# vigor-nf/vigor

Measured on AMD Instinct MI355X. Metric: Mpackets/s device-resident, 64B vignat @1M flows; %HBM roofline, higher is better.
Workload: dtype u8; 1 GPU; vignat 64B, 1M flows, 1xMI355X (parse+hash+map-probe kernel, checksum rewrite); flows=1048576, batch_packets_per_gpu=16777216, global_batch_packets=16777216, frame_bytes=60, slot_bytes=64, order=rr, port=one per burst (vp_dev_batch.in_port), parallelism=single

## Files before the change

vigor_amd/csrc/vp_internal.h:

```cpp
#pragma once

#include <hip/hip_ext.h>
#include <hip/hip_runtime.h>
#include <stdint.h>
#include <stdlib.h>
#include <string.h>

#include <mutex>
#include <tuple>
#include <vector>

#include "../../include/vigpath.h"
#include "vp_device.h"

#define VP_HIP(call)                                                      \
  do {                                                                    \
    hipError_t e_ = (call);                                               \
    if (e_ != hipSuccess) return vp::hip_fail(e_, #call, __FILE__, __LINE__); \
  } while (0)

#define VP_TRY(call)          \
  do {                        \
    int rc_ = (call);         \
    if (rc_) return rc_;      \
// ... 111 lines not shown
  uint32_t sh_live;
  uint32_t own_new;
  uint32_t run_tiles;
  uint32_t last_first;
};

constexpr int kPubGath = 5;
struct CtlPub {
  Ctl ctl;
  uint32_t xtra[(kPubGath + 1) * 64];
  uint32_t epoch;
};

struct JournalCtl {
  uint32_t tail, cnt;
  int64_t floor;
};
constexpr int64_t kJournalNone = INT64_MAX;

struct FlowTable {
  Bucket *bk = nullptr;
  uint32_t bmask = 0;
  uint32_t cap = 0;
  uint32_t mix = 0;
  uint64_t ins_since = 0;
  uint32_t layout_tries = 0;
  uint64_t rebuilds = 0;
  uint32_t *lin = nullptr;
  uint32_t lin_ok = 0;
  bool lin_tried = false;
  uint64_t nb_nominal = 0;
  uint64_t nb_base = 0;
  uint32_t *slot_of = nullptr;
  uint32_t *hash_of = nullptr;
  uint64_t *ts = nullptr;
  uint64_t *tseq = nullptr;
  uint64_t *birth = nullptr;
  uint32_t *stack = nullptr;
  uint32_t *lastg = nullptr;
  Ctl *ctl = nullptr;
  Ctl h_ctl{};
  Ctl *h_pin = nullptr;
  CtlPub *h_pub = nullptr;
  CtlPub *d_pub = nullptr;
  uint32_t pub_epoch = 0;
  uint32_t *ttotal = nullptr;
  uint64_t ts_floor = UINT64_MAX;
  uint32_t fs_hint = 0;
  bool runs_seen = true;
  uint32_t last_run_tiles = 0;
  bool ctl_clean = false;
  uint64_t *ekey = nullptr, *ekey2 = nullptr;
  uint32_t *eidx = nullptr, *eidx2 = nullptr;
  JournalCtl *jr = nullptr;
  uint4 *jrec = nullptr;
  uint32_t jr_n = 0;
  bool jr_on = false;
  uint4 *kv = nullptr;
  uint32_t own_n = 0, own_r = 0;
};

struct CallBuf {
  void *p = nullptr;
  size_t bytes = 0;
  hipEvent_t ev = nullptr;
  hipStream_t last = nullptr;
  bool used = false;
};
int callbuf_reserve(CallBuf &w, size_t bytes, hipStream_t s);
inline int callbuf_done(CallBuf &w, hipStream_t s) {
  VP_HIP(hipEventRecord(w.ev, s));
  w.used = true;
  w.last = s;
  return 0;
}

struct Workspace {
  uint32_t cap_n = 0;
  uint32_t *miss = nullptr;
  uint32_t *miss_sorted = nullptr;
  uint32_t *defer = nullptr;
  uint32_t *reprobe = nullptr;
  uint32_t *reprobe_cnt = nullptr;
  uint32_t *missq = nullptr;
  uint32_t *mkey = nullptr;
  uint32_t *pairs = nullptr;
  uint16_t *in_fill = nullptr;
  size_t in_fill_n = 0;
  CallBuf tx_cnt, txp_sum, rxu_sum, rxm_rec;
  unsigned long long *nkset = nullptr;
  size_t nkset_n = 0;
  uint32_t nk_tag = 0;
  uint32_t *nkbits = nullptr, *nkpre = nullptr, *nkfirst = nullptr, *nkcnt = nullptr;
  size_t nkbits_n = 0, nkfirst_n = 0;
  uint4 *mkq = nullptr;
  uint32_t *mhq = nullptr;
  uint32_t *mhash = nullptr;
  uint32_t *first = nullptr;
  uint32_t *rank = nullptr;
  uint32_t *rep = nullptr;
  uint32_t *assign = nullptr;
  uint32_t *scratch = nullptr;
  uint32_t *log = nullptr;
  uint32_t *log2 = nullptr;
  uint32_t *defer_sorted = nullptr;
  uint32_t *aux = nullptr, *aux_sorted = nullptr;
// ... 252 lines not shown
```

vigor_amd/csrc/vp_table.hip:

```cpp
#include <hip/hip_runtime.h>

#include <cstddef>
#include <hipcub/hipcub.hpp>
#include <unistd.h>

#include <algorithm>
#include <cstdio>
#include <cstdlib>
#include <cstring>
#include <mutex>
#include <vector>

#include "vp_comm.h"
#include "vp_table.h"

namespace vp {

VP_PRELOAD_UNIT(table)


uint32_t grid_for(uint64_t n, uint32_t block, uint32_t max_blocks) {
  uint64_t g = (n + block - 1) / block;
  if (g == 0) g = 1;
  return (uint32_t)(g < max_blocks ? g : max_blocks);
// ... 62 lines not shown
  return 0;
}

int read_ctl_wait(vp_ctx *c, FlowTable &t) {
  hipError_t e;
  while ((e = hipEventQuery(c->evc)) == hipErrorNotReady) {
  }
  VP_HIP(e);
  t.h_ctl = *t.h_pin;
  return 0;
}

int read_ctl2_post(vp_ctx *c, FlowTable &a, FlowTable &b) {
  VP_HIP(hipMemcpyAsync(a.h_pin, a.ctl, sizeof(Ctl), hipMemcpyDeviceToHost,
                        c->stream));
  VP_HIP(hipMemcpyAsync(b.h_pin, b.ctl, sizeof(Ctl), hipMemcpyDeviceToHost,
                        c->stream));
  VP_HIP(hipEventRecord(c->evc, c->stream));
  return 0;
}

int read_ctl2_wait(vp_ctx *c, FlowTable &a, FlowTable &b) {
  hipError_t e;
  while ((e = hipEventQuery(c->evc)) == hipErrorNotReady) {
  }
  VP_HIP(e);
  a.h_ctl = *a.h_pin;
  b.h_ctl = *b.h_pin;
  return 0;
}

int read_ctl2(vp_ctx *c, FlowTable &a, FlowTable &b) {
  VP_HIP(hipMemcpyAsync(a.h_pin, a.ctl, sizeof(Ctl), hipMemcpyDeviceToHost,
                        c->stream));
  VP_HIP(hipMemcpyAsync(b.h_pin, b.ctl, sizeof(Ctl), hipMemcpyDeviceToHost,
                        c->stream));
  VP_HIP(stream_wait(c->stream));
  a.h_ctl = *a.h_pin;
  b.h_ctl = *b.h_pin;
  return 0;
}

TableDev tbl_dev(const FlowTable &t) {
  return TableDev{t.bk,  t.bmask, t.cap,   t.mix, t.slot_of, t.hash_of, t.ts,
                  t.tseq, t.birth, t.stack, t.ctl, t.kv,      t.own_n,   t.own_r,
                  t.lin};
}

template <class T>
static int dalloc(T **p, size_t count) {
  if (count == 0) count = 1;
  hipError_t e = hipMalloc((void **)p, sizeof(T) * count);
  return e == hipSuccess ? 0 : hip_fail(e, "hipMalloc", __FILE__, __LINE__);
}

static int tbl_rebuild(vp_ctx *c, FlowTable &t, uint64_t nb_new = 0);
static int tbl_choose_layout(vp_ctx *c, FlowTable &t);
static int tbl_try_linear(vp_ctx *c, FlowTable &t);
__global__ void lay_count(TableDev t, uint32_t mix, uint32_t *cnt);
__global__ void lay_score(const uint32_t *cnt, uint32_t nb, uint32_t *over);

static uint64_t tbl_entries(const FlowTable &t) {
  return (uint64_t)(t.bmask + 1) * kBucketEntries;
}

uint32_t tbl_initial_mix() {
  const char *mix = getenv("VIGPATH_MIX");
  return mix && atoi(mix) ? kMixMul : 0;
}

int tbl_alloc(vp_ctx *c, FlowTable &t, uint32_t cap) {
  (void)c;
  uint64_t nb = 64;
  while (nb < cap) nb <<= 1;
  t.nb_base = nb;
  int k = 1;
  if (const char *sp = getenv("VIGPATH_SPARSE")) k = atoi(sp);
  if (k > 0) nb <<= std::min(k, 3);
  if (k < 0) nb = std::max<uint64_t>(64, nb >> std::min(-k, 3));
  t.bmask = (uint32_t)(nb - 1);
  t.nb_nominal = nb;
  t.cap = cap;
  t.mix = tbl_initial_mix();
  VP_TRY(dalloc(&t.bk, nb));
  VP_TRY(dalloc(&t.slot_of, cap));
  VP_TRY(dalloc(&t.hash_of, cap));
  VP_TRY(dalloc(&t.ts, cap));
  VP_TRY(dalloc(&t.tseq, cap));
  VP_TRY(dalloc(&t.birth, cap));
  VP_TRY(dalloc(&t.stack, cap));
  VP_TRY(dalloc(&t.lastg, cap));
  VP_TRY(dalloc(&t.ctl, 1));
  VP_HIP(hipHostMalloc((void **)&t.h_pin, sizeof(Ctl), hipHostMallocDefault));
  VP_HIP(hipHostMalloc((void **)&t.h_pub, sizeof(CtlPub),
                       hipHostMallocMapped | hipHostMallocCoherent));
  memset(t.h_pub, 0, sizeof(CtlPub));
  VP_HIP(hipHostGetDevicePointer((void **)&t.d_pub, t.h_pub, 0));
  VP_TRY(dalloc(&t.ttotal, 1));
  VP_TRY(dalloc(&t.ekey, cap));
  VP_TRY(dalloc(&t.ekey2, cap));
  VP_TRY(dalloc(&t.eidx, cap));
  VP_TRY(dalloc(&t.eidx2, cap));
  VP_HIP(hipMemset(t.bk, 0xFF, sizeof(Bucket) * nb));
  VP_HIP(hipMemset(t.slot_of, 0xFF, sizeof(uint32_t) * (size_t)cap));
  VP_HIP(hipMemset(t.ts, 0, sizeof(uint64_t) * (size_t)cap));
  VP_HIP(hipMemset(t.tseq, 0, sizeof(uint64_t) * (size_t)cap));
  VP_HIP(hipMemset(t.birth, 0, sizeof(uint64_t) * (size_t)cap));
  VP_HIP(hipMemset(t.ctl, 0, sizeof(Ctl)));
  t.ts_floor = ~0ull;
  return 0;
}

void tbl_free(FlowTable &t) {
  void *ptrs[] = {t.bk,    t.slot_of, t.hash_of, t.ts,    t.tseq,
                  t.birth, t.stack,   t.lastg,   t.ctl,   t.ekey,
                  t.ekey2, t.eidx,    t.eidx2};
  for (void *p : ptrs) hipFree(p);
  hipFree(t.ttotal);
  hipFree(t.lin);
  hipFree(t.kv);
  hipFree(t.jr);
  hipFree(t.jrec);
  if (t.h_pin) hipHostFree(t.h_pin);
  if (t.h_pub) hipHostFree(t.h_pub);
  t = FlowTable{};
}


struct NkArgs {
  TableDev t;
  const uint32_t *pos;
  uint32_t n;
  uint32_t *mkey, *mhash, *first, *rank, *rep, *assign, *scratch;
  uint32_t smask;
  uint64_t seq_base;
};

__global__ void nk_dedup(NkArgs m) {
  for (uint32_t j = blockIdx.x * blockDim.x + threadIdx.x; j < m.n;
       j += gridDim.x * blockDim.x) {
    const uint32_t *kj = m.mkey + 4 * (size_t)j;
    uint32_t s = home_bucket(m.mhash[j], m.smask, kMixMul);
    for (;;) {
      uint32_t old = atomicCAS(&m.scratch[s], kEmpty, j);
      if (old == kEmpty) break;
      const uint32_t *ko = m.mkey + 4 * (size_t)old;
      if (m.mhash[old] == m.mhash[j] && key_eq(ko, kj)) {
        if (j < old) atomicMin(&m.scratch[s], j);
        break;
      }
      s = (s + 1) & m.smask;
    }
    m.rep[j] = s;
  }
}

__global__ void nk_first(NkArgs m) {
  for (uint32_t j = blockIdx.x * blockDim.x + threadIdx.x; j < m.n;
       j += gridDim.x * blockDim.x)
    m.first[j] = m.scratch[m.rep[j]] == j ? 1u : 0u;
}

__global__ void nk_alloc(NkArgs m) {
  const TableDev &t = m.t;
  const uint32_t stack_top = t.ctl->stack_top;
  const uint32_t fresh = t.ctl->fresh_next;
  const uint32_t free_total = stack_top + (t.cap - fresh);
  uint32_t disp = 0, ins = 0;
  for (uint32_t j = blockIdx.x * blockDim.x + threadIdx.x; j < m.n;
       j += gridDim.x * blockDim.x) {
    if (!m.first[j]) continue;
// ... 7 lines not shown
    const uint32_t *key = m.mkey + 4 * (size_t)j;
    const bool mine = !t.own_n || owner_of(m.mhash[j], t.own_n) == t.own_r;
    uint32_t e = kElsewhere;
    if (mine) {
      bool tomb = false;
      e = tbl_insert(t, m.mhash[j], key, idx, &tomb, &disp);
      if (tomb) atomicAdd(&t.ctl->tomb_reused, 1u);
      ins++;
    }
    if (t.kv) t.kv[idx] = make_uint4(key[0], key[1], key[2], key[3]);
    t.slot_of[idx] = e;
    t.hash_of[idx] = m.mhash[j];
    t.birth[idx] = m.seq_base + m.pos[j];
    m.assign[j] = idx;
  }
  for (uint32_t o = 32; o > 0; o >>= 1) {
    disp += __shfl_xor(disp, o);
    ins += __shfl_xor(ins, o);
  }
  if ((threadIdx.x & 63) == 0 && disp) atomicAdd(&t.ctl->disp_count, disp);
  if ((threadIdx.x & 63) == 0 && ins) atomicAdd(&t.ctl->sh_live, ins);
}

__global__ void nk_commit(NkArgs m) {
  if (threadIdx.x != 0 || blockIdx.x != 0) return;
  Ctl *c = m.t.ctl;
  const uint32_t K = m.rank[m.n - 1] + m.first[m.n - 1];
  const uint32_t free_total = c->stack_top + (m.t.cap - c->fresh_next);
  const uint32_t used = K < free_total ? K : free_total;
  if (used <= c->stack_top) {
    c->stack_top -= used;
  } else {
    c->fresh_next += used - c->stack_top;
    c->stack_top = 0;
  }
  c->n_live += used;
  c->n_tomb -= c->tomb_reused;
  c->tomb_reused = 0;
  c->new_count = used;
}

struct NkuArgs {
  TableDev t;
  const uint32_t *pos;
  const uint4 *key;
  const uint32_t *hash;
  const uint32_t *sq;
  const uint4 *skey;
  const uint32_t *shash;
  uint32_t n, smask;
  unsigned long long *set;
  uint32_t tag;
  uint32_t *rep, *bits, *pre, *first, *cnt;
  uint32_t p0, nwords;
  NowSpec now;
  uint64_t seq_base;
};

__device__ __forceinline__ uint32_t nku_pos(const NkuArgs &m, uint32_t j) {
  const uint32_t e = m.pos[j];
  return e & kMissSlice ? m.sq[e & ~kMissSlice] : e;
}
__device__ __forceinline__ uint4 nku_key(const NkuArgs &m, uint32_t j) {
  const uint32_t e = m.pos[j];
  return e & kMissSlice ? m.skey[e & ~kMissSlice] : m.key[j];
}
__device__ __forceinline__ uint32_t nku_hash(const NkuArgs &m, uint32_t j) {
  const uint32_t e = m.pos[j];
  return e & kMissSlice ? m.shash[e & ~kMissSlice] : m.hash[j];
}

__global__ void nku_dedup(NkuArgs m) {
  const size_t S = (size_t)m.smask + 1;
  unsigned long long *ord = m.set, *fp = m.set + S, *lp = m.set + 2 * S;
  const unsigned long long tg = (unsigned long long)m.tag << 32;
  for (uint32_t j = blockIdx.x * blockDim.x + threadIdx.x; j < m.n;
       j += gridDim.x * blockDim.x) {
    const uint4 kj = nku_key(m, j);
    const uint32_t h = nku_hash(m, j);
    uint32_t s = home_bucket(h, m.smask, kMixMul);
    for (;;) {
      unsigned long long cur = ord[s];
      if ((cur >> 32) != m.tag) {
        const unsigned long long old = atomicCAS(&ord[s], cur, tg | j);
        if (old == cur) break;
        cur = old;
      }
      const uint32_t o = (uint32_t)cur;
      const uint4 ko = nku_key(m, o);
      if (nku_hash(m, o) == h && ko.x == kj.x && ko.y == kj.y && ko.z == kj.z && ko.w == kj.w)
        break;
      s = (s + 1) & m.smask;
    }
    m.rep[j] = s;
    const uint32_t p = nku_pos(m, j);
    const unsigned long long f = tg | (unsigned long long)(~p), l = tg | (unsigned long long)p;
    if (f > fp[s]) atomicMax(&fp[s], f);
    if (l > lp[s]) atomicMax(&lp[s], l);
  }
}

__global__ void nku_firsts(NkuArgs m) {
  const size_t S = (size_t)m.smask + 1;
  const unsigned long long *fp = m.set + S;
  for (uint32_t j = blockIdx.x * blockDim.x + threadIdx.x; j < m.n;
       j += gridDim.x * blockDim.x) {
    const uint32_t p = nku_pos(m, j);
    bool f = (uint32_t)~(uint32_t)fp[m.rep[j]] == p;
    if (f) {
      const uint32_t bit = 1u << ((p - m.p0) & 31);
      f = !(atomicOr(&m.bits[(p - m.p0) >> 5], bit) & bit);
    }
    if (f) atomicMax(&m.t.ctl->last_first, p - m.p0 + 1);
    const uint32_t k = wave_append(m.cnt, f);
    if (f) m.first[k] = j;
  }
}

__global__ void nku_popc(const uint32_t *bits, uint32_t n, uint32_t *out) {
  for (uint32_t i = blockIdx.x * blockDim.x + threadIdx.x; i < n; i += gridDim.x * blockDim.x)
    out[i] = (uint32_t)__popc(bits[i]);
}

__global__ void nku_alloc(NkuArgs m) {
  const TableDev &t = m.t;
  const size_t S = (size_t)m.smask + 1;
  const unsigned long long *lp = m.set + 2 * S;
  const uint32_t stack_top = t.ctl->stack_top;
  const uint32_t fresh = t.ctl->fresh_next;
  const uint32_t free_total = stack_top + (t.cap - fresh);
  const uint32_t K = *m.cnt;
  uint32_t disp = 0, ins = 0;
  for (uint32_t f = blockIdx.x * blockDim.x + threadIdx.x; f < K;
       f += gridDim.x * blockDim.x) {
    const uint32_t j = m.first[f];
    const uint32_t p = nku_pos(m, j), q = p - m.p0, s = m.rep[j];
    const uint32_t r = m.pre[q >> 5] + (uint32_t)__popc(m.bits[q >> 5] & ((1u << (q & 31)) - 1u));
    unsigned long long *ord = m.set;
    const unsigned long long tg = (unsigned long long)m.tag << 32;
    if (r >= free_total) {
      ord[s] = tg | kNone;
      continue;
    }
    const uint32_t idx = r < stack_top ? t.stack[stack_top - 1 - r] : fresh + (r - stack_top);
    const uint4 k4 = nku_key(m, j);
    const uint32_t hj = nku_hash(m, j);
    const uint32_t key[4] = {k4.x, k4.y, k4.z, k4.w};
    bool tomb = false;
    const uint32_t e = tbl_insert(t, hj, key, idx, &tomb, &disp);
    if (tomb) atomicAdd(&t.ctl->tomb_reused, 1u);
    ins++;
    t.slot_of[idx] = e;
    t.hash_of[idx] = hj;
    t.birth[idx] = m.seq_base + p;
    const uint32_t last = (uint32_t)lp[s];
    t.ts[idx] = (uint64_t)m.now.at(last);
    t.tseq[idx] = m.seq_base + last;
    ord[s] = tg | idx;
  }
  for (uint32_t o = 32; o > 0; o >>= 1) {
    disp += __shfl_xor(disp, o);
    ins += __shfl_xor(ins, o);
  }
  if ((threadIdx.x & 63) == 0 && disp) atomicAdd(&t.ctl->disp_count, disp);
  if ((threadIdx.x & 63) == 0 && ins) atomicAdd(&t.ctl->sh_live, ins);
}

__global__ void nku_commit(Ctl *c, uint32_t cap, const uint32_t *cnt) {
  if (threadIdx.x != 0 || blockIdx.x != 0) return;
  const uint32_t K = *cnt;
  const uint32_t free_total = c->stack_top + (cap - c->fresh_next);
  const uint32_t used = K < free_total ? K : free_total;
  if (used <= c->stack_top) {
    c->stack_top -= used;
  } else {
    c->fresh_next += used - c->stack_top;
    c->stack_top = 0;
  }
  c->n_live += used;
  c->n_tomb -= c->tomb_reused;
  c->tomb_reused = 0;
  c->new_count = used;
}

static int tbl_after_new_keys(vp_ctx *c, FlowTable &t);

int tbl_new_keys_unsorted(vp_ctx *c, FlowTable &t, uint32_t n, uint32_t p0, uint32_t p1,
                          const NowSpec &now, uint64_t seq_base) {
  Workspace &w = c->ws;
  if (!n) return 0;
  const uint64_t S = next_pow2(2ull * n);
  const uint32_t nwords = (p1 - p0 + 31) / 32;
  if (3 * S > w.nkset_n) {
    VP_HIP(hipStreamSynchronize(c->stream));
    hipFree(w.nkset);
    w.nkset = nullptr;
    w.nkset_n = 0;
    VP_TRY(dalloc(&w.nkset, 3 * S));
    VP_HIP(hipMemsetAsync(w.nkset, 0, 8 * 3 * S, c->stream));
    w.nkset_n = 3 * S;
    w.nk_tag = 0;
  }
  if (nwords + 1 > w.nkbits_n) {
    VP_HIP(hipStreamSynchronize(c->stream));
    for (uint32_t **p : {&w.nkbits, &w.nkpre}) {
      hipFree(*p);
      *p = nullptr;
    }
    w.nkbits_n = 0;
    VP_TRY(dalloc(&w.nkbits, nwords + 1));
    VP_TRY(dalloc(&w.nkpre, nwords + 1));
    w.nkbits_n = nwords + 1;
  }
  if (n > w.nkfirst_n) {
    VP_HIP(hipStreamSynchronize(c->stream));
    hipFree(w.nkfirst);
    w.nkfirst = nullptr;
    w.nkfirst_n = 0;
    VP_TRY(dalloc(&w.nkfirst, n));
    w.nkfirst_n = n;
  }
  if (!w.nkcnt) VP_TRY(dalloc(&w.nkcnt, 1));
  if (++w.nk_tag == 0) {
    VP_HIP(hipMemsetAsync(w.nkset, 0, 8 * w.nkset_n, c->stream));
    w.nk_tag = 1;
  }
  NkuArgs m{};
  m.t = tbl_dev(t);
  m.pos = w.miss;
  m.key = reinterpret_cast<const uint4 *>(w.mkey);
  m.hash = w.mhash;
  m.sq = w.missq;
  m.skey = w.mkq;
  m.shash = w.mhq;
  m.n = n;
  m.smask = (uint32_t)(S - 1);
  m.set = w.nkset;
  m.tag = w.nk_tag;
  m.rep = w.rep;
  m.bits = w.nkbits;
  m.pre = w.nkpre;
  m.first = w.nkfirst;
  m.cnt = w.nkcnt;
  m.p0 = p0;
  m.nwords = nwords;
  m.now = now;
  m.seq_base = seq_base;
  size_t need = 0;
  hipcub::DeviceScan::ExclusiveSum(nullptr, need, w.nkpre, w.nkpre, (int)nwords, c->stream);
  VP_TRY(cub_reserve(c, need));
  VP_HIP(hipMemsetAsync(w.nkbits, 0, 4ull * nwords, c->stream));
  VP_HIP(hipMemsetAsync(w.nkcnt, 0, 4, c->stream));
  VP_HIP(hipMemsetAsync(&t.ctl->last_first, 0, 4, c->stream));
  const uint32_t g = grid_for(n);
  nku_dedup<<<g, 256, 0, c->stream>>>(m);
  nku_firsts<<<g, 256, 0, c->stream>>>(m);
  nku_popc<<<grid_for(nwords), 256, 0, c->stream>>>(w.nkbits, nwords, w.nkpre);
  VP_HIP(hipcub::DeviceScan::ExclusiveSum(w.cub_tmp, w.cub_bytes, w.nkpre, w.nkpre,
                                          (int)nwords, c->stream));
  nku_alloc<<<g, 256, 0, c->stream>>>(m);
  nku_commit<<<1, 64, 0, c->stream>>>(t.ctl, t.cap, w.nkcnt);
  VP_HIP(hipGetLastError());
  return 0;
}

int tbl_new_keys_done(vp_ctx *c, FlowTable &t) {
  VP_TRY(read_ctl(c, t));
  return tbl_after_new_keys(c, t);
}

int tbl_new_keys(vp_ctx *c, FlowTable &t, const NewKeys &nk, uint64_t seq_base,
                 uint32_t *n_new) {
  Workspace &w = c->ws;
  NkArgs m{};
  m.t = tbl_dev(t);
  m.pos = nk.pos;
  m.n = nk.n;
  m.mkey = w.mkey;
  m.mhash = w.mhash;
  m.first = w.first;
  m.rank = w.rank;
  m.rep = w.rep;
  m.assign = w.assign;
  m.scratch = w.scratch;
  m.seq_base = seq_base;
  const uint32_t ssize = next_pow2((uint64_t)nk.n * 2);
  m.smask = ssize - 1;
  size_t need = 0;
  hipcub::DeviceScan::ExclusiveSum(nullptr, need, w.first, w.rank, (int)nk.n,
                                   c->stream);
  VP_TRY(cub_reserve(c, need));
  VP_HIP(hipMemsetAsync(w.scratch, 0xFF, sizeof(uint32_t) * (size_t)ssize,
                        c->stream));
  const uint32_t g = grid_for(nk.n);
  nk_dedup<<<g, 256, 0, c->stream>>>(m);
  nk_first<<<g, 256, 0, c->stream>>>(m);
  VP_HIP(hipcub::DeviceScan::ExclusiveSum(w.cub_tmp, w.cub_bytes, w.first,
                                          w.rank, (int)nk.n, c->stream));
  nk_alloc<<<g, 256, 0, c->stream>>>(m);
  nk_commit<<<1, 64, 0, c->stream>>>(m);
  VP_HIP(hipGetLastError());
  VP_TRY(read_ctl(c, t));
  if (n_new) *n_new = t.h_ctl.new_count;
  return tbl_after_new_keys(c, t);
}

static int tbl_after_new_keys(vp_ctx *c, FlowTable &t) {
  t.ins_since += t.h_ctl.new_count;
  if (t.lin_ok && !t.lin_tried && !t.own_n && t.mix != kMixLin &&
      2ull * t.h_ctl.n_live > t.nb_base) {
    VP_TRY(tbl_try_linear(c, t));
    if (t.mix == kMixLin) {
      VP_HIP(hipMemsetAsync(&t.ctl->max_disp, 0, 4, c->stream));
      return 0;
// ... 585 lines not shown
}

__global__ void reprobe_stamp(const uint32_t *list, const uint32_t *cnt, uint32_t n,
                              uint32_t range, uint32_t nblk, const uint32_t *log,
                              NowSpec now, uint64_t seq_base, uint64_t *ts,
                              const uint64_t *tseq) {
  for (uint32_t b = blockIdx.x; b < nblk; b += gridDim.x) {
    const uint32_t nb = reprobe_slice_len(cnt, n, range, b);
    for (uint32_t k = threadIdx.x; k < nb; k += blockDim.x) {
      const uint32_t p = list[(size_t)b * range + k];
      const uint32_t i = log[p];
      if (i != kNone && tseq[i] == seq_base + p) ts[i] = (uint64_t)now.at(p);
    }
  }
}

__global__ void late_max(const uint32_t *list, const uint32_t *cnt, uint32_t n,
                         uint32_t range, uint32_t nblk, const uint32_t *log,
                         uint64_t seq_base, uint64_t *tseq) {
  for (uint32_t b = blockIdx.x; b < nblk; b += gridDim.x) {
    const uint32_t nb = reprobe_slice_len(cnt, n, range, b);
    for (uint32_t k = threadIdx.x; k < nb; k += blockDim.x) {
      const uint32_t p = list[(size_t)b * range + k];
      const uint32_t i = log[p];
      if (i != kNone)
        atomicMax(reinterpret_cast<unsigned long long *>(tseq + i),
                  (unsigned long long)(seq_base + p));
    }
  }
}

int tbl_late_touches(vp_ctx *c, FlowTable &t, const uint32_t *list,
                     const uint32_t *cnt, uint32_t n, uint32_t range, uint32_t nblk,
                     const uint32_t *log, const NowSpec &now, uint64_t seq_base) {
  if (nblk == 0) return 0;
  const uint32_t g = std::min<uint32_t>(nblk, 2048);
  late_max<<<g, 256, 0, c->stream>>>(list, cnt, n, range, nblk, log, seq_base, t.tseq);
  reprobe_stamp<<<g, 256, 0, c->stream>>>(list, cnt, n, range, nblk, log, now,
                                          seq_base, t.ts, t.tseq);
  VP_HIP(hipGetLastError());
  return 0;
}

int tbl_reprobe_stamp(vp_ctx *c, FlowTable &t, const uint32_t *list,
                      const uint32_t *cnt, uint32_t n, uint32_t range, uint32_t nblk,
                      const uint32_t *log, const NowSpec &now, uint64_t seq_base) {
  reprobe_stamp<<<std::min<uint32_t>(nblk, 2048), 256, 0, c->stream>>>(
      list, cnt, n, range, nblk, log, now, seq_base, t.ts, t.tseq);
  VP_HIP(hipGetLastError());
  return 0;
}


__global__ __launch_bounds__(256) void exp_collect(TableDev t, int64_t cutoff, uint64_t *ekey,
                                                   uint32_t *eidx) {
  __shared__ uint32_t cnt, base;
  __shared__ unsigned long long wmin[4];
  if (threadIdx.x == 0) cnt = 0;
  __syncthreads();
  const uint32_t per = (t.cap + gridDim.x - 1) / gridDim.x;
  const uint32_t i0 = blockIdx.x * per, i1 = min(t.cap, i0 + per);
  auto take_at = [&](uint32_t i) { return t.slot_of[i] != kNone && (int64_t)t.ts[i] < cutoff; };
  unsigned long long low = ~0ull;
  for (uint32_t i = i0 + threadIdx.x; i < i1; i += blockDim.x) {
    const bool live = t.slot_of[i] != kNone;
    const uint64_t ts = live ? t.ts[i] : ~0ull;
    const bool take = live && (int64_t)ts < cutoff;
    wave_append(&cnt, take);
    if (live && !take && ts < low) low = ts;
  }
  for (int o = 32; o > 0; o >>= 1) {
    const unsigned long long v = __shfl_xor(low, o);
    low = v < low ? v : low;
  }
  if (__lane_id() == 0) wmin[threadIdx.x >> 6] = low;
  __syncthreads();
  if (threadIdx.x == 0) {
    for (uint32_t w = 1; w < blockDim.x / 64; w++) low = wmin[w] < low ? wmin[w] : low;
    if (low != ~0ull) atomicMin((unsigned long long *)&t.ctl->min_ts, low);
  }
  if (threadIdx.x == 0) {
    base = cnt ? atomicAdd(&t.ctl->exp_count, cnt) : 0u;
    cnt = 0;
  }
  __syncthreads();
  for (uint32_t i = i0 + threadIdx.x; i < i1; i += blockDim.x) {
    const bool take = take_at(i);
    const uint32_t k = base + wave_append(&cnt, take);
    if (take) {
      eidx[k] = i;
      ekey[k] = t.tseq[i];
    }
  }
}

__global__ __launch_bounds__(256) void exp_apply(TableDev t, const uint32_t *eidx, uint32_t n) {
  __shared__ uint32_t tombs;
  if (threadIdx.x == 0) tombs = 0;
  __syncthreads();
  const uint32_t top = t.ctl->stack_top;
  for (uint32_t j = blockIdx.x * blockDim.x + threadIdx.x; j < n;
       j += gridDim.x * blockDim.x) {
    const uint32_t idx = eidx[j];
    const uint32_t e = t.slot_of[idx];
    t.stack[top + j] = idx;
    const bool own = e < kElsewhere;
    if (own) t.bk[e >> 2].idx[e & 3] = kTomb;
    t.slot_of[idx] = kNone;
    wave_append(&tombs, own);
  }
  __syncthreads();
  if (threadIdx.x == 0 && tombs) atomicAdd(&t.ctl->n_tomb, tombs);
}

__global__ void exp_commit(Ctl *ctl, uint32_t n, uint32_t n_tomb_before) {
  if (threadIdx.x == 0 && blockIdx.x == 0) {
    ctl->stack_top += n;
    ctl->n_live -= n;
    ctl->sh_live -= ctl->n_tomb - n_tomb_before;
  }
}

__global__ void rb_collect(TableDev t, uint32_t *keys) {
  for (uint32_t i = blockIdx.x * blockDim.x + threadIdx.x; i < t.cap;
       i += gridDim.x * blockDim.x) {
    if (t.slot_of[i] >= kElsewhere) continue;
    const uint4 k = tbl_key_of(t, i);
    reinterpret_cast<uint4 *>(keys)[i] = k;
  }
}
__global__ void rb_insert(TableDev t, const uint32_t *keys) {
  for (uint32_t i = blockIdx.x * blockDim.x + threadIdx.x; i < t.cap;
       i += gridDim.x * blockDim.x) {
    if (t.slot_of[i] >= kElsewhere) continue;
    bool tomb = false;
    uint32_t disp = 0;
    t.slot_of[i] = tbl_insert(t, t.hash_of[i], keys + 4 * (size_t)i, i, &tomb, &disp);
  }
}

static int tbl_rebuild(vp_ctx *c, FlowTable &t, uint64_t nb_new) {
  t.rebuilds++;
  uint32_t *keys = reinterpret_cast<uint32_t *>(t.kv);
  if (!keys) {
    VP_TRY(dalloc(&keys, 4ull * t.cap));
    rb_collect<<<grid_for(t.cap), 256, 0, c->stream>>>(tbl_dev(t), keys);
  }
  if (nb_new && nb_new != (uint64_t)t.bmask + 1) {
    VP_HIP(hipStreamSynchronize(c->stream));
    VP_HIP(hipFree(t.bk));
    t.bk = nullptr;
    VP_TRY(dalloc(&t.bk, nb_new));
    t.bmask = (uint32_t)(nb_new - 1);
  }
  VP_HIP(hipMemsetAsync(t.bk, 0xFF, sizeof(Bucket) * ((size_t)t.bmask + 1),
                        c->stream));
  rb_insert<<<grid_for(t.cap), 256, 0, c->stream>>>(tbl_dev(t), keys);
  VP_HIP(hipMemsetAsync(&t.ctl->n_tomb, 0, 4, c->stream));
  VP_HIP(hipMemsetAsync(&t.ctl->disp_count, 0, 4, c->stream));
  t.ins_since = 0;
  VP_HIP(hipStreamSynchronize(c->stream));
  if (!t.kv) VP_HIP(hipFree(keys));
  return 0;
}

int tbl_set_owner(vp_ctx *c, FlowTable &t, uint32_t n, uint32_t r) {
  VP_TRY(dalloc(&t.kv, t.cap));
  t.own_n = n;
  t.own_r = r;
  uint64_t nb = 64;
  while (nb * n < t.cap) nb <<= 1;
  return tbl_rebuild(c, t, nb);
}

__global__ void own_count(const uint32_t *mhash, uint32_t n, uint32_t own_n,
                          uint32_t own_r, Ctl *ctl) {
  for (uint32_t j = blockIdx.x * blockDim.x + threadIdx.x; j < n;
       j += gridDim.x * blockDim.x) {
    const uint32_t k = wave_append(&ctl->own_new, owner_of(mhash[j], own_n) == own_r);
    (void)k;
  }
}

int tbl_owner_reserve(vp_ctx *c, FlowTable &t, uint32_t n) {
  if (!t.own_n || !n) return 0;
  VP_HIP(hipMemsetAsync(&t.ctl->own_new, 0, 4, c->stream));
  own_count<<<grid_for(n), 256, 0, c->stream>>>(c->ws.mhash, n, t.own_n, t.own_r,
                                                t.ctl);
  VP_HIP(hipGetLastError());
  VP_TRY(read_ctl(c, t));
  const uint64_t need = (uint64_t)t.h_ctl.sh_live + t.h_ctl.n_tomb + t.h_ctl.own_new;
  if (need <= (uint64_t)t.bmask + 1) return 0;
  uint64_t nb = (uint64_t)t.bmask + 1;
  while (nb < need) nb <<= 1;
  return tbl_rebuild(c, t, nb);
}

int tbl_expire(vp_ctx *c, FlowTable &t, int64_t cutoff, uint32_t *n_out) {
  VP_HIP(hipMemsetAsync(&t.ctl->exp_count, 0, 4, c->stream));
  VP_HIP(hipMemsetAsync(&t.ctl->min_ts, 0xFF, 8, c->stream));
  exp_collect<<<grid_for(t.cap, 256, 512), 256, 0, c->stream>>>(tbl_dev(t), cutoff, t.ekey,
                                                                t.eidx);
  VP_HIP(hipGetLastError());
  VP_TRY(read_ctl(c, t));
  const uint32_t k = t.h_ctl.exp_count;
  t.ts_floor = t.h_ctl.min_ts;
  if (n_out) *n_out = k;
  if (k == 0) return 0;
  VP_TRY(sort_pairs(c, t.ekey, t.ekey2, t.eidx, t.eidx2, k, 64));
  exp_apply<<<grid_for(k), 256, 0, c->stream>>>(tbl_dev(t), t.eidx2, k);
  exp_commit<<<1, 64, 0, c->stream>>>(t.ctl, k, t.h_ctl.n_tomb);
  VP_HIP(hipGetLastError());
  if (t.own_n) return tbl_check_tombs(c, t);
  Ctl &h = t.h_ctl;
  h.stack_top += k;
  h.n_live -= k;
  h.n_tomb += k;
  h.sh_live -= k;
  const uint64_t base = std::min<uint64_t>(tbl_entries(t), t.nb_base * kBucketEntries);
  if ((uint64_t)h.n_tomb + h.sh_live > base * 85 / 100) return tbl_rebuild(c, t);
  return 0;
}

int tbl_check_tombs(vp_ctx *c, FlowTable &t) {
  VP_TRY(read_ctl(c, t));
  const uint64_t base = std::min<uint64_t>(tbl_entries(t), t.nb_base * kBucketEntries);
  if ((uint64_t)t.h_ctl.n_tomb + t.h_ctl.sh_live > base * 85 / 100)
    return tbl_rebuild(c, t);
  return 0;
}

uint32_t tbl_purge_bound(const FlowTable &t) {
  const uint64_t base = std::min<uint64_t>(tbl_entries(t), t.nb_base * kBucketEntries);
  return (uint32_t)std::min<uint64_t>(base * 85 / 100, UINT32_MAX);
}


__global__ void jr_fill(TableDev t, const uint64_t *seq, const uint32_t *idx, uint32_t k,
                        uint4 *rec, JournalCtl *jc) {
  for (uint32_t j = blockIdx.x * blockDim.x + threadIdx.x; j < k; j += gridDim.x * blockDim.x)
    rec[j] = make_uint4((uint32_t)seq[j], (uint32_t)(seq[j] >> 32), idx[j], 0u);
  if (blockIdx.x == 0 && threadIdx.x == 0) {
    jc->tail = 0;
    jc->cnt = k;
    jc->floor = k ? (int64_t)t.ts[idx[0]] : kJournalNone;
  }
}

int tbl_live_collect(vp_ctx *c, FlowTable &t) {
  VP_HIP(hipMemsetAsync(&t.ctl->exp_count, 0, 4, c->stream));
  VP_HIP(hipMemsetAsync(&t.ctl->min_ts, 0xFF, 8, c->stream));
  exp_collect<<<grid_for(t.cap, 256, 512), 256, 0, c->stream>>>(tbl_dev(t), INT64_MAX, t.ekey,
                                                                t.eidx);
  VP_HIP(hipGetLastError());
  return 0;
}

int tbl_live_sort(vp_ctx *c, FlowTable &t, uint32_t k, const uint64_t **seq,
                  const uint32_t **idx) {
  *seq = t.ekey;
  *idx = t.eidx;
  if (k > 1) {
    VP_TRY(sort_pairs(c, t.ekey, t.ekey2, t.eidx, t.eidx2, k, 64));
    *seq = t.ekey2;
    *idx = t.eidx2;
  }
  return 0;
}

int tbl_layout_check(vp_ctx *c, FlowTable &t) {
  VP_TRY(read_ctl(c, t));
  return tbl_after_new_keys(c, t);
}

int tbl_journal_seed(vp_ctx *c, FlowTable &t) {
  if (!t.jr) {
    static const uint32_t mult = [] {
      const char *e = getenv("VIGPATH_SERVE_JOURNAL");
      return (uint32_t)std::min(1024, std::max(2, e ? atoi(e) : 8));
    }();
    const uint64_t n = std::min<uint64_t>((uint64_t)mult * std::max(t.cap, 1u), 1u << 30);
    if (n < 2ull * t.cap) return state_fail("journal: table of %u indices is too large", t.cap);
    VP_TRY(dalloc(&t.jrec, n));
    VP_TRY(dalloc(&t.jr, 1));
    t.jr_n = (uint32_t)n;
  }
  VP_TRY(tbl_live_collect(c, t));
  VP_TRY(read_ctl(c, t));
  const uint32_t k = t.h_ctl.exp_count;
  if (k > t.cap) return state_fail("journal: %u live indices in a table of %u", k, t.cap);
  const uint64_t *seq = nullptr;
  const uint32_t *idx = nullptr;
  VP_TRY(tbl_live_sort(c, t, k, &seq, &idx));
  jr_fill<<<grid_for(std::max(k, 1u)), 256, 0, c->stream>>>(tbl_dev(t), seq, idx, k, t.jrec, t.jr);
  VP_HIP(hipGetLastError());
  VP_HIP(stream_wait(c->stream));
  t.jr_on = true;
  return 0;
}


int ws_reserve(vp_ctx *c, uint32_t n);

int sort_keys(vp_ctx *c, const uint32_t *in, uint32_t *out, uint32_t n) {
  if (!n) return 0;
  size_t need = 0;
// ... 459 lines not shown
```

Measured before the change: 39770 Mpps.

## Replace expiry radix sort with histogram-binned rank-and-apply, fuse new-key scan

Expiry no longer runs a full radix sort of expired sequence keys. exp_collect now builds an adaptive histogram over the sequence numbers, and a single fused kernel uses the histogram prefix sums to bucket each key into a tile, bitonic-sorts the tile in LDS and applies the tombstones. The new-key path replaces popc plus a hipcub scan plus a commit kernel with one decoupled scan kernel, and folds the commit into nku_alloc through a last-block-done pattern. The aim is fewer kernel launches and less sort traffic per batch. In exchange it adds adaptive bin state carried across calls, a fallback to the old path when a bin overflows, and relaxed-atomic ordering subtleties.

```diff
diff --git a/vigor_amd/csrc/vp_internal.h b/vigor_amd/csrc/vp_internal.h
--- a/vigor_amd/csrc/vp_internal.h
+++ b/vigor_amd/csrc/vp_internal.h
@@ -187,6 +187,7 @@
   bool ctl_clean = false;
   uint64_t *ekey = nullptr, *ekey2 = nullptr;
   uint32_t *eidx = nullptr, *eidx2 = nullptr;
+  struct ExpBins *ebins = nullptr;
   JournalCtl *jr = nullptr;
   uint4 *jrec = nullptr;
   uint32_t jr_n = 0;
diff --git a/vigor_amd/csrc/vp_table.hip b/vigor_amd/csrc/vp_table.hip
--- a/vigor_amd/csrc/vp_table.hip
+++ b/vigor_amd/csrc/vp_table.hip
@@ -138,6 +138,27 @@
   if (count == 0) count = 1;
   hipError_t e = hipMalloc((void **)p, sizeof(T) * count);
   return e == hipSuccess ? 0 : hip_fail(e, "hipMalloc", __FILE__, __LINE__);
+}
+
+constexpr uint32_t kExpBins = 2048;
+struct ExpBins {
+  uint32_t hist[kExpBins];
+  uint32_t done_collect, done_apply;
+  uint32_t shift, shift_used;
+  unsigned long long lo, lo_used;
+  unsigned long long span;
+  unsigned long long smax, smin;
+  unsigned long long stay;
+};
+static int exp_bins_alloc(FlowTable &t) {
+  VP_TRY(dalloc(&t.ebins, 1));
+  VP_HIP(hipMemset(t.ebins, 0, sizeof(ExpBins)));
+  const uint32_t shift = 14;
+  const unsigned long long span = (unsigned long long)kExpBins << shift;
+  VP_HIP(hipMemcpy(&t.ebins->shift, &shift, 4, hipMemcpyHostToDevice));
+  VP_HIP(hipMemcpy(&t.ebins->span, &span, 8, hipMemcpyHostToDevice));
+  VP_HIP(hipMemset(&t.ebins->smin, 0xFF, 16));
+  return 0;
 }
 
 static int tbl_rebuild(vp_ctx *c, FlowTable &t, uint64_t nb_new = 0);
@@ -187,6 +208,7 @@
   VP_TRY(dalloc(&t.ekey2, cap));
   VP_TRY(dalloc(&t.eidx, cap));
   VP_TRY(dalloc(&t.eidx2, cap));
+  VP_TRY(exp_bins_alloc(t));
   VP_HIP(hipMemset(t.bk, 0xFF, sizeof(Bucket) * nb));
   VP_HIP(hipMemset(t.slot_of, 0xFF, sizeof(uint32_t) * (size_t)cap));
   VP_HIP(hipMemset(t.ts, 0, sizeof(uint64_t) * (size_t)cap));
@@ -203,6 +225,7 @@
                   t.ekey2, t.eidx,    t.eidx2};
   for (void *p : ptrs) hipFree(p);
   hipFree(t.ttotal);
+  hipFree(t.ebins);
   hipFree(t.lin);
   hipFree(t.kv);
   hipFree(t.jr);
@@ -316,10 +339,49 @@
   unsigned long long *set;
   uint32_t tag;
   uint32_t *rep, *bits, *pre, *first, *cnt;
+  uint32_t *cbase;
+  uint32_t *done;
   uint32_t p0, nwords;
   NowSpec now;
   uint64_t seq_base;
 };
+
+__device__ __forceinline__ bool last_block_done(uint32_t *counter) {
+  __shared__ uint32_t last;
+  asm volatile("s_waitcnt vmcnt(0)" ::: "memory");
+  __syncthreads();
+  if (threadIdx.x == 0)
+    last = __hip_atomic_fetch_add(counter, 1u, __ATOMIC_RELAXED, __HIP_MEMORY_SCOPE_AGENT) ==
+           gridDim.x - 1;
+  __syncthreads();
+  return last != 0;
+}
+__device__ __forceinline__ uint32_t dev_load(const uint32_t *p) {
+  return __hip_atomic_load(p, __ATOMIC_RELAXED, __HIP_MEMORY_SCOPE_AGENT);
+}
+__device__ __forceinline__ void dev_store(uint32_t *p, uint32_t v) {
+  __hip_atomic_store(p, v, __ATOMIC_RELAXED, __HIP_MEMORY_SCOPE_AGENT);
+}
+
+__device__ __forceinline__ uint32_t block_excl_scan(uint32_t v, uint32_t *ws, uint32_t *total) {
+  const uint32_t lane = __lane_id(), w = threadIdx.x >> 6, nw = blockDim.x >> 6;
+  uint32_t inc = v;
+  for (uint32_t o = 1; o < 64; o <<= 1) {
+    const uint32_t u = __shfl_up(inc, o);
+    if (lane >= o) inc += u;
+  }
+  __syncthreads();
+  if (lane == 63) ws[w] = inc;
+  __syncthreads();
+  uint32_t off = 0, tot = 0;
+  for (uint32_t i = 0; i < nw; i++) {
+    const uint32_t x = ws[i];
+    if (i < w) off += x;
+    tot += x;
+  }
+  *total = tot;
+  return off + inc - v;
+}
 
 __device__ __forceinline__ uint32_t nku_pos(const NkuArgs &m, uint32_t j) {
   const uint32_t e = m.pos[j];
@@ -381,9 +443,39 @@
   }
 }
 
-__global__ void nku_popc(const uint32_t *bits, uint32_t n, uint32_t *out) {
-  for (uint32_t i = blockIdx.x * blockDim.x + threadIdx.x; i < n; i += gridDim.x * blockDim.x)
-    out[i] = (uint32_t)__popc(bits[i]);
+constexpr uint32_t kNkuChunk = 2048;
+__global__ __launch_bounds__(256) void nku_scan(const uint32_t *bits, uint32_t nwords,
+                                                uint32_t *pre, uint32_t *cbase, uint32_t *done) {
+  __shared__ uint32_t ws[16];
+  const uint32_t w0 = blockIdx.x * kNkuChunk + threadIdx.x * 8;
+  uint32_t v[8];
+  if (w0 + 8 <= nwords) {
+    const uint4 a = *reinterpret_cast<const uint4 *>(bits + w0);
+    const uint4 b = *reinterpret_cast<const uint4 *>(bits + w0 + 4);
+    v[0] = a.x, v[1] = a.y, v[2] = a.z, v[3] = a.w;
+    v[4] = b.x, v[5] = b.y, v[6] = b.z, v[7] = b.w;
+  } else {
+    for (uint32_t i = 0; i < 8; i++) v[i] = w0 + i < nwords ? bits[w0 + i] : 0u;
+  }
+  uint32_t sum = 0;
+  for (uint32_t i = 0; i < 8; i++) sum += (uint32_t)__popc(v[i]);
+  uint32_t total;
+  uint32_t at = block_excl_scan(sum, ws, &total);
+  for (uint32_t i = 0; i < 8; i++) {
+    if (w0 + i < nwords) pre[w0 + i] = at;
+    at += (uint32_t)__popc(v[i]);
+  }
+  if (threadIdx.x == 0) dev_store(&cbase[blockIdx.x], total);
+  if (!last_block_done(done)) return;
+  uint32_t carry = 0;
+  for (uint32_t c0 = 0; c0 < gridDim.x; c0 += blockDim.x) {
+    const uint32_t i = c0 + threadIdx.x;
+    const uint32_t x = i < gridDim.x ? dev_load(&cbase[i]) : 0u;
+    const uint32_t e = block_excl_scan(x, ws, &total);
+    if (i < gridDim.x) cbase[i] = carry + e;
+    carry += total;
+  }
+  if (threadIdx.x == 0) dev_store(done, 0u);
 }
 
 __global__ void nku_alloc(NkuArgs m) {
@@ -399,7 +491,8 @@
        f += gridDim.x * blockDim.x) {
     const uint32_t j = m.first[f];
     const uint32_t p = nku_pos(m, j), q = p - m.p0, s = m.rep[j];
-    const uint32_t r = m.pre[q >> 5] + (uint32_t)__popc(m.bits[q >> 5] & ((1u << (q & 31)) - 1u));
+    const uint32_t r = m.cbase[(q >> 5) / kNkuChunk] + m.pre[q >> 5] +
+                       (uint32_t)__popc(m.bits[q >> 5] & ((1u << (q & 31)) - 1u));
     unsigned long long *ord = m.set;
     const unsigned long long tg = (unsigned long long)m.tag << 32;
     if (r >= free_total) {
@@ -428,23 +521,20 @@
   }
   if ((threadIdx.x & 63) == 0 && disp) atomicAdd(&t.ctl->disp_count, disp);
   if ((threadIdx.x & 63) == 0 && ins) atomicAdd(&t.ctl->sh_live, ins);
-}
-
-__global__ void nku_commit(Ctl *c, uint32_t cap, const uint32_t *cnt) {
-  if (threadIdx.x != 0 || blockIdx.x != 0) return;
-  const uint32_t K = *cnt;
-  const uint32_t free_total = c->stack_top + (cap - c->fresh_next);
+  if (!last_block_done(&m.done[1]) || threadIdx.x != 0) return;
+  Ctl *c = t.ctl;
   const uint32_t used = K < free_total ? K : free_total;
-  if (used <= c->stack_top) {
-    c->stack_top -= used;
+  if (used <= stack_top) {
+    c->stack_top = stack_top - used;
   } else {
-    c->fresh_next += used - c->stack_top;
+    c->fresh_next = fresh + (used - stack_top);
     c->stack_top = 0;
   }
   c->n_live += used;
-  c->n_tomb -= c->tomb_reused;
-  c->tomb_reused = 0;
+  c->n_tomb -= dev_load(&c->tomb_reused);
+  dev_store(&c->tomb_reused, 0u);
   c->new_count = used;
+  dev_store(&m.done[1], 0u);
 }
 
 static int tbl_after_new_keys(vp_ctx *c, FlowTable &t);
@@ -473,7 +563,7 @@
     }
     w.nkbits_n = 0;
     VP_TRY(dalloc(&w.nkbits, nwords + 1));
-    VP_TRY(dalloc(&w.nkpre, nwords + 1));
+    VP_TRY(dalloc(&w.nkpre, (size_t)nwords + 1 + (nwords + 1) / kNkuChunk + 2));
     w.nkbits_n = nwords + 1;
   }
   if (n > w.nkfirst_n) {
@@ -484,7 +574,10 @@
     VP_TRY(dalloc(&w.nkfirst, n));
     w.nkfirst_n = n;
   }
-  if (!w.nkcnt) VP_TRY(dalloc(&w.nkcnt, 1));
+  if (!w.nkcnt) {
+    VP_TRY(dalloc(&w.nkcnt, 4));
+    VP_HIP(hipMemsetAsync(w.nkcnt, 0, 16, c->stream));
+  }
   if (++w.nk_tag == 0) {
     VP_HIP(hipMemsetAsync(w.nkset, 0, 8 * w.nkset_n, c->stream));
     w.nk_tag = 1;
@@ -506,24 +599,21 @@
   m.pre = w.nkpre;
   m.first = w.nkfirst;
   m.cnt = w.nkcnt;
+  m.cbase = w.nkpre + w.nkbits_n;
+  m.done = w.nkcnt + 1;
   m.p0 = p0;
   m.nwords = nwords;
   m.now = now;
   m.seq_base = seq_base;
-  size_t need = 0;
-  hipcub::DeviceScan::ExclusiveSum(nullptr, need, w.nkpre, w.nkpre, (int)nwords, c->stream);
-  VP_TRY(cub_reserve(c, need));
   VP_HIP(hipMemsetAsync(w.nkbits, 0, 4ull * nwords, c->stream));
   VP_HIP(hipMemsetAsync(w.nkcnt, 0, 4, c->stream));
   VP_HIP(hipMemsetAsync(&t.ctl->last_first, 0, 4, c->stream));
   const uint32_t g = grid_for(n);
   nku_dedup<<<g, 256, 0, c->stream>>>(m);
   nku_firsts<<<g, 256, 0, c->stream>>>(m);
-  nku_popc<<<grid_for(nwords), 256, 0, c->stream>>>(w.nkbits, nwords, w.nkpre);
-  VP_HIP(hipcub::DeviceScan::ExclusiveSum(w.cub_tmp, w.cub_bytes, w.nkpre, w.nkpre,
-                                          (int)nwords, c->stream));
+  nku_scan<<<(nwords + kNkuChunk - 1) / kNkuChunk, 256, 0, c->stream>>>(w.nkbits, nwords, w.nkpre,
+                                                                        m.cbase, m.done);
   nku_alloc<<<g, 256, 0, c->stream>>>(m);
-  nku_commit<<<1, 64, 0, c->stream>>>(t.ctl, t.cap, w.nkcnt);
   VP_HIP(hipGetLastError());
   return 0;
 }
@@ -1215,46 +1305,131 @@
 }
 
 
+constexpr uint32_t kExpTile = 1024;
+constexpr uint32_t kExpLds = 4096;
+constexpr uint32_t kExpUnfused = 0x80000000u;
+static uint32_t g_exp_fused_max = 1u << 17;
+extern "C" uint32_t vp_internal_expiry_fused_max(uint32_t k) {
+  const uint32_t was = g_exp_fused_max;
+  g_exp_fused_max = k;
+  return was;
+}
+
+__device__ __forceinline__ uint32_t exp_bin(unsigned long long key, unsigned long long lo,
+                                            uint32_t shift) {
+  if (key <= lo) return 0;
+  const unsigned long long b = (key - lo) >> shift;
+  return b < kExpBins ? (uint32_t)b : kExpBins - 1;
+}
+
 __global__ __launch_bounds__(256) void exp_collect(TableDev t, int64_t cutoff, uint64_t *ekey,
-                                                   uint32_t *eidx) {
+                                                   uint32_t *eidx, ExpBins *eb) {
   __shared__ uint32_t cnt, base;
   __shared__ unsigned long long wmin[4];
+  __shared__ uint32_t wmin_i[4];
+  __shared__ uint32_t lh[kExpBins];
   if (threadIdx.x == 0) cnt = 0;
+  if (eb)
+    for (uint32_t b = threadIdx.x; b < kExpBins; b += blockDim.x) lh[b] = 0;
   __syncthreads();
   const uint32_t per = (t.cap + gridDim.x - 1) / gridDim.x;
   const uint32_t i0 = blockIdx.x * per, i1 = min(t.cap, i0 + per);
   auto take_at = [&](uint32_t i) { return t.slot_of[i] != kNone && (int64_t)t.ts[i] < cutoff; };
   unsigned long long low = ~0ull;
+  uint32_t low_i = 0;
   for (uint32_t i = i0 + threadIdx.x; i < i1; i += blockDim.x) {
     const bool live = t.slot_of[i] != kNone;
     const uint64_t ts = live ? t.ts[i] : ~0ull;
     const bool take = live && (int64_t)ts < cutoff;
     wave_append(&cnt, take);
-    if (live && !take && ts < low) low = ts;
+    if (live && !take && ts < low) low = ts, low_i = i;
   }
   for (int o = 32; o > 0; o >>= 1) {
     const unsigned long long v = __shfl_xor(low, o);
-    low = v < low ? v : low;
-  }
-  if (__lane_id() == 0) wmin[threadIdx.x >> 6] = low;
+    const uint32_t vi = __shfl_xor(low_i, o);
+    if (v < low) low = v, low_i = vi;
+  }
+  if (__lane_id() == 0) wmin[threadIdx.x >> 6] = low, wmin_i[threadIdx.x >> 6] = low_i;
   __syncthreads();
   if (threadIdx.x == 0) {
-    for (uint32_t w = 1; w < blockDim.x / 64; w++) low = wmin[w] < low ? wmin[w] : low;
+    for (uint32_t w = 1; w < blockDim.x / 64; w++)
+      if (wmin[w] < low) low = wmin[w], low_i = wmin_i[w];
     if (low != ~0ull) atomicMin((unsigned long long *)&t.ctl->min_ts, low);
+    if (eb && low != ~0ull) atomicMin(&eb->stay, (unsigned long long)t.tseq[low_i]);
   }
   if (threadIdx.x == 0) {
     base = cnt ? atomicAdd(&t.ctl->exp_count, cnt) : 0u;
     cnt = 0;
   }
   __syncthreads();
+  const unsigned long long lo = eb ? eb->lo : 0ull;
+  const uint32_t shift = eb ? eb->shift : 0u;
+  unsigned long long top = 0, low2 = ~0ull;
   for (uint32_t i = i0 + threadIdx.x; i < i1; i += blockDim.x) {
     const bool take = take_at(i);
     const uint32_t k = base + wave_append(&cnt, take);
     if (take) {
+      const unsigned long long q = t.tseq[i];
       eidx[k] = i;
-      ekey[k] = t.tseq[i];
-    }
-  }
+      ekey[k] = q;
+      if (eb) {
+        atomicAdd(&lh[exp_bin(q, lo, shift)], 1u);
+        top = q > top ? q : top;
+        low2 = q < low2 ? q : low2;
+      }
+    }
+  }
+  if (!eb) return;
+  __syncthreads();
+  for (uint32_t b = threadIdx.x; b < kExpBins; b += blockDim.x)
+    if (lh[b]) atomicAdd(&eb->hist[b], lh[b]);
+  for (int o = 32; o > 0; o >>= 1) {
+    const unsigned long long v = __shfl_xor(top, o);
+    top = v > top ? v : top;
+  }
+  for (int o = 32; o > 0; o >>= 1) {
+    const unsigned long long v = __shfl_xor(low2, o);
+    low2 = v < low2 ? v : low2;
+  }
+  if (__lane_id() == 0 && low2 != ~0ull) {
+    atomicMax(&eb->smax, top);
+    atomicMin(&eb->smin, low2);
+  }
+  if (!last_block_done(&eb->done_collect)) return;
+  __shared__ uint32_t most;
+  if (threadIdx.x == 0) most = 0;
+  __syncthreads();
+  uint32_t mx = 0;
+  for (uint32_t b = threadIdx.x; b < kExpBins; b += blockDim.x) mx = max(mx, dev_load(&eb->hist[b]));
+  for (int o = 32; o > 0; o >>= 1) mx = max(mx, (uint32_t)__shfl_xor(mx, o));
+  if (__lane_id() == 0) atomicMax(&most, mx);
+  __syncthreads();
+  if (threadIdx.x != 0) return;
+  eb->lo_used = lo;
+  eb->shift_used = shift;
+  if (most + kExpTile > kExpLds) atomicOr(&t.ctl->exp_count, kExpUnfused);
+  const unsigned long long stay =
+      __hip_atomic_load(&eb->stay, __ATOMIC_RELAXED, __HIP_MEMORY_SCOPE_AGENT);
+  __hip_atomic_store(&eb->stay, ~0ull, __ATOMIC_RELAXED, __HIP_MEMORY_SCOPE_AGENT);
+  if (most) {
+    const unsigned long long smax =
+        __hip_atomic_load(&eb->smax, __ATOMIC_RELAXED, __HIP_MEMORY_SCOPE_AGENT);
+    const unsigned long long smin =
+        __hip_atomic_load(&eb->smin, __ATOMIC_RELAXED, __HIP_MEMORY_SCOPE_AGENT);
+    const unsigned long long took = smax - smin + 1;
+    unsigned long long span = eb->span >> 1;
+    if (span > 32 * took) span = 32 * took;
+    if (span < 2 * took) span = 2 * took;
+    if (span < kExpBins) span = kExpBins;
+    uint32_t s = 0;
+    while ((span >> s) >= kExpBins) s++;
+    eb->lo = stay != ~0ull && stay > smax ? stay : smax + 1;
+    eb->span = span;
+    eb->shift = s;
+    __hip_atomic_store(&eb->smax, 0ull, __ATOMIC_RELAXED, __HIP_MEMORY_SCOPE_AGENT);
+    __hip_atomic_store(&eb->smin, ~0ull, __ATOMIC_RELAXED, __HIP_MEMORY_SCOPE_AGENT);
+  }
+  dev_store(&eb->done_collect, 0u);
 }
 
 __global__ __launch_bounds__(256) void exp_apply(TableDev t, const uint32_t *eidx, uint32_t n) {
@@ -1282,6 +1457,108 @@
     ctl->n_live -= n;
     ctl->sh_live -= ctl->n_tomb - n_tomb_before;
   }
+}
+
+__global__ __launch_bounds__(1024) void exp_rank_apply(TableDev t, const uint64_t *ekey,
+                                                       const uint32_t *eidx, uint32_t n,
+                                                       ExpBins *eb, uint32_t n_tomb_before) {
+  __shared__ unsigned long long skey[kExpLds];
+  __shared__ uint32_t sidx[kExpLds];
+  __shared__ uint32_t pre[kExpBins];
+  __shared__ uint32_t ws[16];
+  __shared__ uint32_t s_base, s_end, s_cnt, tombs;
+  static_assert(kExpBins == 2 * 1024, "two bins per thread");
+  const uint32_t tid = threadIdx.x;
+  const uint32_t r0 = blockIdx.x * kExpTile, r1 = r0 + kExpTile;
+  {
+    const uint32_t a = eb->hist[2 * tid], b = eb->hist[2 * tid + 1];
+    uint32_t total;
+    const uint32_t e = block_excl_scan(a + b, ws, &total);
+    pre[2 * tid] = e;
+    pre[2 * tid + 1] = e + a;
+  }
+  if (tid == 0) s_base = n, s_end = n, s_cnt = 0, tombs = 0;
+  __syncthreads();
+  for (uint32_t b = 2 * tid; b < 2 * tid + 2; b++) {
+    const uint32_t p = pre[b], q = b ? pre[b - 1] : 0u;
+    if (p >= r0 && (b == 0 || q < r0)) s_base = p;
+    if (p >= r1 && (b == 0 || q < r1)) s_end = p;
+  }
+  __syncthreads();
+  const uint32_t base = s_base;
+  const uint32_t want = base < r1 ? min(s_end, n) - base : 0u;
+  const unsigned long long lo = eb->lo_used;
+  const uint32_t shift = eb->shift_used;
+  if (want) {
+    constexpr uint32_t kU = 8;
+    for (uint32_t i0 = 0; i0 < n; i0 += kU * blockDim.x) {
+      unsigned long long key[kU];
+#pragma unroll
+      for (uint32_t u = 0; u < kU; u++) {
+        const uint32_t i = i0 + u * blockDim.x + tid;
+        key[u] = i < n ? ekey[i] : 0ull;
+      }
+#pragma unroll
+      for (uint32_t u = 0; u < kU; u++) {
+        const uint32_t i = i0 + u * blockDim.x + tid;
+        bool mine = false;
+        if (i < n) {
+          const uint32_t p = pre[exp_bin(key[u], lo, shift)];
+          mine = p >= r0 && p < r1;
+        }
+        const uint32_t k = wave_append(&s_cnt, mine);
+        if (mine && k < kExpLds) {
+          skey[k] = key[u];
+          sidx[k] = eidx[i];
+        }
+      }
+    }
+  }
+  __syncthreads();
+  const uint32_t m = min(s_cnt, kExpLds);
+  uint32_t m2 = 1;
+  while (m2 < m) m2 <<= 1;
+  for (uint32_t i = m + tid; i < m2; i += blockDim.x) skey[i] = ~0ull, sidx[i] = ~0u;
+  __syncthreads();
+  for (uint32_t k = 2; k <= m2; k <<= 1) {
+    for (uint32_t j = k >> 1; j > 0; j >>= 1) {
+      for (uint32_t i = tid; i < m2; i += blockDim.x) {
+        const uint32_t l = i ^ j;
+        if (l > i) {
+          const unsigned long long ka = skey[i], kb = skey[l];
+          const uint32_t ia = sidx[i], ib = sidx[l];
+          const bool gt = ka > kb || (ka == kb && ia > ib);
+          if (gt == ((i & k) == 0)) {
+            skey[i] = kb, skey[l] = ka;
+            sidx[i] = ib, sidx[l] = ia;
+          }
+        }
+      }
+      __syncthreads();
+    }
+  }
+  const uint32_t top = t.ctl->stack_top;
+  for (uint32_t i = tid; i < m; i += blockDim.x) {
+    const uint32_t idx = sidx[i];
+    const uint32_t e = t.slot_of[idx];
+    if (base + i >= n) break;
+    t.stack[top + base + i] = idx;
+    const bool own = e < kElsewhere;
+    if (own) t.bk[e >> 2].idx[e & 3] = kTomb;
+    t.slot_of[idx] = kNone;
+    wave_append(&tombs, own);
+  }
+  __syncthreads();
+  if (tid == 0 && tombs) atomicAdd(&t.ctl->n_tomb, tombs);
+  if (!last_block_done(&eb->done_apply)) return;
+  eb->hist[2 * tid] = 0;
+  eb->hist[2 * tid + 1] = 0;
+  if (tid != 0) return;
+  Ctl *ctl = t.ctl;
+  ctl->stack_top = top + n;
+  ctl->n_live -= n;
+  ctl->sh_live -= dev_load(&ctl->n_tomb) - n_tomb_before;
+  dev_store(&eb->done_apply, 0u);
 }
 
 __global__ void rb_collect(TableDev t, uint32_t *keys) {
@@ -1362,17 +1639,26 @@
 int tbl_expire(vp_ctx *c, FlowTable &t, int64_t cutoff, uint32_t *n_out) {
   VP_HIP(hipMemsetAsync(&t.ctl->exp_count, 0, 4, c->stream));
   VP_HIP(hipMemsetAsync(&t.ctl->min_ts, 0xFF, 8, c->stream));
+  ExpBins *eb = t.cap < kExpUnfused ? t.ebins : nullptr;
   exp_collect<<<grid_for(t.cap, 256, 512), 256, 0, c->stream>>>(tbl_dev(t), cutoff, t.ekey,
-                                                                t.eidx);
+                                                                t.eidx, eb);
   VP_HIP(hipGetLastError());
   VP_TRY(read_ctl(c, t));
+  const bool even = eb && !(t.h_ctl.exp_count & kExpUnfused);
+  if (eb) t.h_ctl.exp_count &= ~kExpUnfused;
   const uint32_t k = t.h_ctl.exp_count;
   t.ts_floor = t.h_ctl.min_ts;
   if (n_out) *n_out = k;
   if (k == 0) return 0;
-  VP_TRY(sort_pairs(c, t.ekey, t.ekey2, t.eidx, t.eidx2, k, 64));
-  exp_apply<<<grid_for(k), 256, 0, c->stream>>>(tbl_dev(t), t.eidx2, k);
-  exp_commit<<<1, 64, 0, c->stream>>>(t.ctl, k, t.h_ctl.n_tomb);
+  if (even && k <= g_exp_fused_max) {
+    exp_rank_apply<<<(k + kExpTile - 1) / kExpTile, 1024, 0, c->stream>>>(
+        tbl_dev(t), t.ekey, t.eidx, k, eb, t.h_ctl.n_tomb);
+  } else {
+    if (eb) VP_HIP(hipMemsetAsync(eb->hist, 0, sizeof eb->hist, c->stream));
+    VP_TRY(sort_pairs(c, t.ekey, t.ekey2, t.eidx, t.eidx2, k, 64));
+    exp_apply<<<grid_for(k), 256, 0, c->stream>>>(tbl_dev(t), t.eidx2, k);
+    exp_commit<<<1, 64, 0, c->stream>>>(t.ctl, k, t.h_ctl.n_tomb);
+  }
   VP_HIP(hipGetLastError());
   if (t.own_n) return tbl_check_tombs(c, t);
   Ctl &h = t.h_ctl;
@@ -1414,7 +1700,7 @@
   VP_HIP(hipMemsetAsync(&t.ctl->exp_count, 0, 4, c->stream));
   VP_HIP(hipMemsetAsync(&t.ctl->min_ts, 0xFF, 8, c->stream));
   exp_collect<<<grid_for(t.cap, 256, 512), 256, 0, c->stream>>>(tbl_dev(t), INT64_MAX, t.ekey,
-                                                                t.eidx);
+                                                                t.eidx, nullptr);
   VP_HIP(hipGetLastError());
   return 0;
 }
```

Measured after the change: 39760 Mpps. About the same (-0.0%).
